# impromptuRong/hd_yolo

Hardware: AMD Instinct MI355X
Metric: tiles/sec (640x640) fwd+bwd (higher is better)
Workload: dtype bf16; 1 GPU; metayolo yolov5s 8-class nuclei, 640x640 RGB tiles, batch 64/GPU, train step = fwd + DetLoss + bwd + all-reduce + SGD(nesterov); global_batch=64, parallelism=dp1, world_size=1, backend=none, hw_queues=4

## Files before the change

### hd_yolo_amd/build.py

```python
import os
import subprocess
import sys
from concurrent.futures import ThreadPoolExecutor

HERE = os.path.dirname(os.path.abspath(__file__))
CSRC = os.path.join(HERE, 'csrc')
OUT = os.path.join(CSRC, 'build')
LIB = os.path.join(OUT, 'libhdyolo_hip.so')
SOURCES = ['api.hip', 'conv_dispatch.hip', 'conv_igemm.hip', 'conv3x3.hip', 'conv3x3_c128.hip', 'conv3x3s2.hip', 'conv_deep.hip', 'conv_stem.hip', 'conv_wgrad.hip', 'conv_wgrad3x3.hip', 'conv_wgrad_deep.hip', 'conv_dgrad_s2.hip', 'conv1x1_bwd.hip', 'bn_act.hip', 'pool.hip', 'detect.hip', 'nms_grid.hip', 'slide.hip', 'augment.hip', 'augment_masks.hip', 'score.hip', 'paste.hip', 'mask_score.hip', 'measure.hip', 'spatial.hip', 'outline.hip', 'graph.hip', 'loss.hip', 'roi.hip', 'seg.hip', 'optim.hip', 'exec.hip']
FLAGS = ['--offload-arch=gfx950', '-O3', '-fPIC', '-std=c++17', '-ffp-contract=off', '-Wall', '-Wno-unused-function',
         '-I' + CSRC, '-I' + os.path.join(os.path.dirname(HERE), 'include')]


def _newer(a, bs):
    return os.path.exists(a) and all(os.path.getmtime(a) >= os.path.getmtime(b) for b in bs)


def build(force=False, verbose=True):
    os.makedirs(OUT, exist_ok=True)
    headers = [os.path.join(CSRC, h) for h in os.listdir(CSRC) if h.endswith('.h')]
    headers += [os.path.join(os.path.dirname(HERE), 'include', h) for h in ('hdyolo.h', 'hdyolo_measure.h', 'hdyolo_spatial.h', 'hdyolo_outline.h', 'hdyolo_graph.h')]
    hipcc = os.environ.get('HIPCC', '/opt/rocm/bin/hipcc')

    def compile_one(src):
        s = os.path.join(CSRC, src)
        o = os.path.join(OUT, src.replace('.hip', '.o'))
        if not force and _newer(o, [s] + headers):
            return o
        cmd = [hipcc] + FLAGS + ['-c', s, '-o', o]
        if verbose:
            print(' '.join(cmd), flush=True)
        subprocess.check_call(cmd)
        return o

    with ThreadPoolExecutor(max_workers=min(6, os.cpu_count() or 1)) as ex:
        objs = list(ex.map(compile_one, SOURCES))
    if force or not _newer(LIB, objs):
        cmd = [hipcc, '--offload-arch=gfx950', '-shared', '-fPIC', '-o', LIB] + objs
        if verbose:
            print(' '.join(cmd), flush=True)
        subprocess.check_call(cmd)
    return LIB


if __name__ == '__main__':
    print(build(force='--force' in sys.argv))
```

### hd_yolo_amd/csrc/api.hip

```cpp
#include <stdarg.h>
#include <stdio.h>
#include <stdlib.h>
#include <string.h>

#include <atomic>

#include "common.h"
#include "hdyolo_internal.h"
#include "hdyolo.h"

int hdy_pack_weight_launch(const hdy_pack_desc& d, hipStream_t st);
int hdy_pack_batch_launch(const hdy_pack_desc* table, int n, int total_blocks, hipStream_t st);

static thread_local char g_err[512] = "";

void hdy_set_error(const char* fmt, ...) {
    va_list ap;
    va_start(ap, fmt);
    vsnprintf(g_err, sizeof(g_err), fmt, ap);
    va_end(ap);
}

namespace {
struct OptDef { const char* name; int def; bool flag; };
const OptDef g_opt_def[HDY_OPT_COUNT] = {
    {"HDY_NO_CLASS_WALK", 0, true}, {"HDY_NO_CONV3X3", 0, true}, {"HDY_C3_GRID", 0, false}, {"HDY_NO_CONV3X3S2", 0, false},
    {"HDY_NO_DGRAD_S2", 0, false}, {"HDY_TILE_INTERLEAVE", 1, false}, {"HDY_NO_BIG_TILES", 0, true}, {"HDY_NO_STEM_KERNEL", 0, true},
    {"HDY_WGRAD_BLOCKS", 512, false}, {"HDY_NO_STEM_WGRAD", 0, true}, {"HDY_NO_WGRAD3X3", 0, true}, 
    {"HDY_LOSS_GRID", 2048, false}, {"HDY_NO_DEEP", 0, true}, {"HDY_NO_WGRAD_DEEP", 0, true}, {"HDY_DEEP_BN", 0, false}, {"HDY_DEEP_DEBUG", 0, false}, {"HDY_DEEP_ALL", 1, false}, {"HDY_DEEP_MIN_TILES", 160, false}, {"HDY_DEEP_WALK", 2, false}, {"HDY_NO_BN_REDUCE4", 0, true},
    {"HDY_WGRAD_TILE", 0, false}, {"HDY_SPPF_NO_KEYS", 0, true}, {"HDY_WGRAD_DEEP_KMIN", 192, false}, {"HDY_NO_CONV3X3_C128", 0, true}, {"HDY_NO_F1X1_96", 0, true},
    {"HDY_AP_CHUNK", 0, false}, {"HDY_AP_NO_PRUNE", 0, true},
};
std::atomic<int> g_opt[HDY_OPT_COUNT];
std::once_flag g_opt_once;
void opt_init() {
    std::call_once(g_opt_once, [] {
        for (int i = 0; i < HDY_OPT_COUNT; ++i) {
            const char* v = getenv(g_opt_def[i].name);
            g_opt[i].store(v ? (g_opt_def[i].flag ? 1 : atoi(v)) : g_opt_def[i].def, std::memory_order_relaxed);
        }
    });
}
int opt_index(const char* name) {
    for (int i = 0; name && i < HDY_OPT_COUNT; ++i)
        if (!strcmp(name, g_opt_def[i].name)) return i;
    return -1;
}
thread_local char g_disp_last[64] = "";
std::mutex g_disp_mu;
char g_disp_log[32768] = "";
size_t g_disp_len = 0;
thread_local char g_disp_copy[32768] = "";
}

int hdy_opt(int id) {
    opt_init();
    return g_opt[id].load(std::memory_order_relaxed);
}

void hdy_note_dispatch(const char* what) {
    snprintf(g_disp_last, sizeof(g_disp_last), "%s", what);
    const size_t n = strlen(g_disp_last);
    std::lock_guard<std::mutex> lock(g_disp_mu);
    if (g_disp_len + n + 2 < sizeof(g_disp_log)) {
        memcpy(g_disp_log + g_disp_len, g_disp_last, n);
        g_disp_log[g_disp_len + n] = ';';
        g_disp_log[g_disp_len + n + 1] = 0;
        g_disp_len += n + 1;
    }
}

namespace {

enum { KIND_FWD = 0, KIND_DGRAD = 1, KIND_STEM = 2 };

inline int velems(int dtype) { return dtype == HDY_BF16 ? 8 : 4; }
inline int bke(int dtype) { return 8 * velems(dtype); }
inline size_t esize(int dtype) { return dtype == HDY_BF16 ? 2 : 4; }

inline size_t block_elems(int rows, int kd, int dtype) {
    const int bn = hdy_conv_bn_tile(rows);
    return (size_t)round_up(rows, bn) * round_up(kd, bke(dtype));
}

}

extern "C" {

const char* hdy_last_error(void) { return g_err; }

const char* hdy_last_dispatch(void) { return g_disp_last; }

const char* hdy_dispatch_log(void) {
    std::lock_guard<std::mutex> lock(g_disp_mu);
    memcpy(g_disp_copy, g_disp_log, g_disp_len + 1);
    return g_disp_copy;
}

void hdy_dispatch_log_reset(void) {
    std::lock_guard<std::mutex> lock(g_disp_mu);
    g_disp_log[0] = 0;
    g_disp_len = 0;
    g_disp_last[0] = 0;
}

int hdy_set_option(const char* name, int value) {
    const int i = opt_index(name);
    HDY_ARG(i >= 0, "set_option: unknown option %s", name ? name : "(null)");
    opt_init();
    return g_opt[i].exchange(value, std::memory_order_relaxed);
}

int hdy_get_option(const char* name) {
    const int i = opt_index(name);
    HDY_ARG(i >= 0, "get_option: unknown option %s", name ? name : "(null)");
    return hdy_opt(i);
}

int hdy_version(void) { return HDY_ABI_VERSION; }

int hdy_fastdiv_magic(unsigned d, unsigned* magic, int* shift) {
    HDY_ARG(d > 0 && magic && shift, "fastdiv_magic: d must be positive");
    hdy_magic(d, magic, shift);
    return HDY_OK;
}

int hdy_conv_out_dim(int in, int k, int stride, int pad) { return conv_out_dim(in, k, stride, pad); }

int hdy_conv_mtiles(long long M) { return (int)((M + 127) / 128); }

size_t hdy_conv_pack_elems(int K, int C, int R, int S, int stride, int pad, int kind, int dtype) {
    if (kind == KIND_FWD) return block_elems(K, R * S * C, dtype);
    if (kind == KIND_STEM) return block_elems(K, R * S * 4, dtype);
    if (stride == 1) return block_elems(C, R * S * K, dtype);
    size_t n = 0;
    for (int a = 0; a < 2; ++a)
        for (int b = 0; b < 2; ++b) {
            const Axis ah = class_axis(R, pad, a), aw = class_axis(S, pad, b);
            if (ah.taps && aw.taps) n += block_elems(C, ah.taps * aw.taps * K, dtype);
        }
    return n;
}

static hdy_pack_desc make_desc(const float* w_a, int K_a, const float* w_b, int K_b, void* out, int Kl, int C, int R, int S, int transpose,
                               int TH, int TW, int rbase, int rstep, int sbase, int sstep, int stem, int rows_total, int Kdp, int dtype,
                               int first_block) {
    hdy_pack_desc d = {};
    d.w_a = w_a; d.w_b = w_b; d.out = out; d.K_a = K_a; d.K_b = K_b; d.Kl = Kl; d.C = C; d.R = R; d.S = S; d.transpose = transpose;
    d.TH = TH; d.TW = TW; d.rbase = rbase; d.rstep = rstep; d.sbase = sbase; d.sstep = sstep; d.stem = stem; d.rows_total = rows_total;
    d.Kdp = Kdp; d.dtype = dtype; d.first_block = first_block;
    d.nblocks = cdiv((long long)rows_total * Kdp, 2048);
    return d;
}

int hdy_conv_pack_describe(const float* w_a, int K_a, const float* w_b, int K_b, int K, int C, int R, int S, int stride, int pad, int kind,
                           int dtype, void* out, hdy_pack_desc* descs, int first_block) {
    HDY_ARG(w_a && out && descs && K_a > 0 && K_b >= 0 && K >= K_a + K_b && C > 0 && R > 0 && S > 0, "conv_pack: bad args");
    HDY_ARG((K_b == 0) == (w_b == nullptr), "conv_pack: w_b / K_b mismatch");
    HDY_ARG(stride == 1 || stride == 2, "conv_pack: stride %d unsupported", stride);
    HDY_ARG(dtype == HDY_BF16 || dtype == HDY_F32, "conv_pack: unknown dtype %d", dtype);
    HDY_ARG(((long long)K + 256) * ((long long)R * S * ((long long)C + 256) + 64) < (1LL << 31), "conv_pack: weight too large for 32-bit packing indices");
    if (kind == KIND_FWD || kind == KIND_STEM) {
        const int stem = kind == KIND_STEM;
        HDY_ARG(!stem || (C == 3 && K_b == 0), "conv_pack: stem expects C == 3 and a single weight");
        const int kd = stem ? R * S * 4 : R * S * C;
        const int Kdp = round_up(kd, bke(dtype));
        const int rows_total = round_up(K, hdy_conv_bn_tile(K));
        descs[0] = make_desc(w_a, K_a, w_b, K_b, out, K, C, R, S, 0, R, stem ? 1 : S, 0, 1, 0, 1, stem, rows_total, Kdp, dtype, first_block);
        return 1;
    }
    HDY_ARG(kind == KIND_DGRAD, "conv_pack: unknown kind %d", kind);
    const int rows_total = round_up(C, hdy_conv_bn_tile(C));
    if (stride == 1) {
        const int Kdp = round_up(R * S * K, bke(dtype));
        descs[0] = make_desc(w_a, K_a, w_b, K_b, out, K, C, R, S, 1, R, S, R - 1, -1, S - 1, -1, 0, rows_total, Kdp, dtype, first_block);
        return 1;
    }
    size_t off = 0;
    int n = 0;
    for (int a = 0; a < 2; ++a)
        for (int b = 0; b < 2; ++b) {
            const Axis ah = class_axis(R, pad, a), aw = class_axis(S, pad, b);
            if (!ah.taps || !aw.taps) continue;
            const int Kdp = round_up(ah.taps * aw.taps * K, bke(dtype));
// ... 28 lines not shown
```

### hd_yolo_amd/csrc/common.h

```cpp
#pragma once
#include <hip/hip_runtime.h>
#include <stdint.h>
#include <stddef.h>

#include <mutex>

#define HDY_OK 0
#define HDY_EINVAL (-1)
#define HDY_EUNSUPPORTED (-2)

enum { HDY_F32 = 0, HDY_BF16 = 1 };

void hdy_set_error(const char* fmt, ...);

enum HdyOption {
    HDY_OPT_NO_CLASS_WALK,
    HDY_OPT_NO_CONV3X3,
    HDY_OPT_C3_GRID,
    HDY_OPT_NO_CONV3X3S2,
    HDY_OPT_NO_DGRAD_S2,
    HDY_OPT_TILE_INTERLEAVE,
    HDY_OPT_NO_BIG_TILES,
    HDY_OPT_NO_STEM_KERNEL,
    HDY_OPT_WGRAD_BLOCKS,
    HDY_OPT_NO_STEM_WGRAD,
    HDY_OPT_NO_WGRAD3X3,
    HDY_OPT_LOSS_GRID,
    HDY_OPT_NO_DEEP,
    HDY_OPT_NO_WGRAD_DEEP,
    HDY_OPT_DEEP_BN,
    HDY_OPT_DEEP_DEBUG,
    HDY_OPT_DEEP_ALL,
    HDY_OPT_DEEP_MIN_TILES,
    HDY_OPT_DEEP_WALK,
    HDY_OPT_NO_BN_REDUCE4,
    HDY_OPT_WGRAD_TILE,
    HDY_OPT_SPPF_NO_KEYS,
    HDY_OPT_WGRAD_DEEP_KMIN,
    HDY_OPT_NO_CONV3X3_C128,
    HDY_OPT_NO_F1X1_96,
    HDY_OPT_AP_CHUNK,
    HDY_OPT_AP_NO_PRUNE,
    HDY_OPT_COUNT
};
int hdy_opt(int id);

void hdy_note_dispatch(const char* what);

#define HDY_ARG(cond, ...)                 \
    do {                                   \
        if (!(cond)) {                     \
            hdy_set_error(__VA_ARGS__);    \
            return HDY_EINVAL;             \
        }                                  \
    } while (0)

#define HDY_LAUNCH_CHECK(what)                                                       \
    do {                                                                             \
        hipError_t e__ = hipGetLastError();                                          \
        if (e__ != hipSuccess) {                                                     \
            hdy_set_error("%s: launch failed: %s", what, hipGetErrorString(e__));    \
            return (int)e__;                                                         \
        }                                                                            \
    } while (0)

typedef __bf16 bf16_t;
typedef int i32x4 __attribute__((ext_vector_type(4)));
typedef float f32x4 __attribute__((ext_vector_type(4)));
typedef __bf16 bf16x8 __attribute__((ext_vector_type(8)));
typedef __bf16 bf16x4 __attribute__((ext_vector_type(4)));

#if defined(__HIPCC__)
__device__ __forceinline__ float row_sum16(float v) {
#ifdef HDY_ROW_SUM_SHFL
    for (int m = 1; m < 16; m <<= 1) v += __shfl_xor(v, m);
    return v;
#endif
    v += __builtin_bit_cast(float, __builtin_amdgcn_update_dpp(0, __builtin_bit_cast(int, v), 0x128, 0xF, 0xF, true));
    v += __builtin_bit_cast(float, __builtin_amdgcn_update_dpp(0, __builtin_bit_cast(int, v), 0x124, 0xF, 0xF, true));
    v += __builtin_bit_cast(float, __builtin_amdgcn_update_dpp(0, __builtin_bit_cast(int, v), 0x122, 0xF, 0xF, true));
    v += __builtin_bit_cast(float, __builtin_amdgcn_update_dpp(0, __builtin_bit_cast(int, v), 0x121, 0xF, 0xF, true));
    return v;
}
#endif

struct PerDeviceOnce {
    std::once_flag flag[16];
    template <typename F> void run(F&& fn) {
        int dev = 0;
        (void)hipGetDevice(&dev);
        std::call_once(flag[dev & 15], fn);
    }
};

static inline int cdiv(long long a, long long b) { return (int)((a + b - 1) / b); }
static inline int round_up(int a, int b) { return (a + b - 1) / b * b; }

#ifdef __HIPCC__
union V16 {
    i32x4 i;
    f32x4 f;
    bf16x8 h;
};

__device__ __forceinline__ float silu_f(float u) { return u / (1.0f + __expf(-u)); }
__device__ __forceinline__ float sigmoid_f(float u) { return 1.0f / (1.0f + __expf(-u)); }

template <typename T> __device__ __forceinline__ float to_f32(T v);
template <> __device__ __forceinline__ float to_f32<float>(float v) { return v; }
template <> __device__ __forceinline__ float to_f32<bf16_t>(bf16_t v) { return (float)v; }
template <typename T> __device__ __forceinline__ T from_f32(float v);
template <> __device__ __forceinline__ float from_f32<float>(float v) { return v; }
template <> __device__ __forceinline__ bf16_t from_f32<bf16_t>(float v) { return (bf16_t)v; }

__device__ __forceinline__ int xcd_remap(int id, int n) {
    const int q = n >> 3, r = n & 7, x = id & 7, s = id >> 3;
    return (x < r ? x * (q + 1) : r * (q + 1) + (x - r) * q) + s;
}
__device__ __forceinline__ unsigned fdiv(unsigned n, unsigned mg, int sh) { return __umulhi(n << 1, mg) >> sh; }

__device__ __forceinline__ bool iou_gt(float ax1, float ay1, float ax2, float ay2, float aarea, float bx1, float by1, float bx2, float by2,
                                       float barea, float thr) {
    const float xx1 = ax1 > bx1 ? ax1 : bx1;
    const float yy1 = ay1 > by1 ? ay1 : by1;
    const float xx2 = ax2 < bx2 ? ax2 : bx2;
    const float yy2 = ay2 < by2 ? ay2 : by2;
    float w = __fsub_rn(xx2, xx1);
    float h = __fsub_rn(yy2, yy1);
    w = w < 0.f ? 0.f : w;
    h = h < 0.f ? 0.f : h;
    const float inter = __fmul_rn(w, h);
    const float ovr = __fdiv_rn(inter, __fsub_rn(__fadd_rn(aarea, barea), inter));
    return ovr > thr;
}

__device__ __forceinline__ unsigned desc_key(float s) {
    unsigned u = s == 0.0f ? 0u : __float_as_uint(s);
    u = (u & 0x80000000u) ? ~u : (u | 0x80000000u);
    return ~u;
}

__device__ __forceinline__ void glds16(const void* g, unsigned char* lds_wave_base) {
    __builtin_amdgcn_global_load_lds((const void __attribute__((address_space(1)))*)g,
                                     (void __attribute__((address_space(3)))*)lds_wave_base, 16, 0, 0);
}

__device__ __forceinline__ void lds_dma16(__amdgpu_buffer_rsrc_t r, unsigned voff, unsigned soff, unsigned char* lds_wave_base) {
    __builtin_amdgcn_raw_ptr_buffer_load_lds(r, (void __attribute__((address_space(3)))*)lds_wave_base, 16, (int)voff, (int)soff, 0, 0);
}

__device__ __forceinline__ void lds_dma16(__amdgpu_buffer_rsrc_t r, unsigned voff, unsigned soff, unsigned lds_byte) {
    __builtin_amdgcn_raw_ptr_buffer_load_lds(r, (void __attribute__((address_space(3)))*)(uintptr_t)lds_byte, 16, (int)voff, (int)soff, 0, 0);
}

__device__ __forceinline__ int fsw(int row) { return ((row >> 1) & 1) | (((row >> 3) & 1) << 1); }
__device__ __forceinline__ int fsw3(int row) { return (row & 6) ^ (((row >> 3) & 1) * 5); }

__device__ __forceinline__ float fast_sigmoid(float u) { return __builtin_amdgcn_rcpf(1.0f + __expf(-u)); }
__device__ __forceinline__ float dsilu_f(float u) {
    const float s = fast_sigmoid(u);
    return s * (1.0f + u * (1.0f - s));
}

template <typename T> __device__ __forceinline__ void unpack(const i32x4& v, float* f);
template <> __device__ __forceinline__ void unpack<float>(const i32x4& v, float* f) {
    V16 u; u.i = v;
#pragma unroll
    for (int i = 0; i < 4; ++i) f[i] = u.f[i];
}
template <> __device__ __forceinline__ void unpack<bf16_t>(const i32x4& v, float* f) {
    V16 u; u.i = v;
#pragma unroll
    for (int i = 0; i < 8; ++i) f[i] = (float)u.h[i];
}
template <typename T> __device__ __forceinline__ i32x4 pack(const float* f);
template <> __device__ __forceinline__ i32x4 pack<float>(const float* f) {
    V16 u;
#pragma unroll
    for (int i = 0; i < 4; ++i) u.f[i] = f[i];
    return u.i;
}
template <> __device__ __forceinline__ i32x4 pack<bf16_t>(const float* f) {
    V16 u;
#pragma unroll
    for (int i = 0; i < 8; ++i) u.h[i] = (bf16_t)f[i];
    return u.i;
}

#define VEC_OK(ptr, ld, VE) ((((uintptr_t)(ptr)) & 15) == 0 && (ld) % (VE) == 0)

#define S2_LDSR(dst, addr)                                                                             \
    do {                                                                                               \
        if constexpr (HAND) asm volatile("ds_read_b128 %0, %1" : "=v"(dst) : "v"(addr) : "memory");    \
        else dst = *(const i32x4*)(smem + ((addr) - lds0));                                            \
    } while (0)
// ... 11 lines not shown
```

### hd_yolo_amd/csrc/conv_dispatch.hip

```cpp
#include "common.h"
#include "hdyolo_internal.h"
#include "hdyolo.h"

static inline int bke(int dtype) { return dtype == HDY_BF16 ? 64 : 32; }

static ConvPlan conv_fwd_plan(const ConvShape& s, int first = CONV_STEM) {
    ConvPlan p = {};
    if (first <= CONV_STEM && hdy_conv_stem_plan(s, &p)) return p;
    if (first <= CONV_3X3_C64 && hdy_conv3x3_c64_plan(s, &p)) return p;
    if (first <= CONV_3X3_C128 && hdy_conv3x3_c128_plan(s, &p)) return p;
    if (first <= CONV_3X3S2 && hdy_conv3x3s2_plan(s, &p)) return p;
    if (first <= CONV_DGRAD_S2 && hdy_dgrad3x3s2_plan(s, &p)) return p;
    if (first <= CONV_DEEP && hdy_conv_deep_plan(s, &p)) return p;
    hdy_conv_igemm_plan(s, &p);
    return p;
}

extern "C" int hdy_conv_stat_slabs(int N, int H, int W, int C, int K, int R, int S, int stride, int pad, int dtype) {
    const int stem = C == 3 && R == 6 && S == 6 && stride == 2 && pad == 2;
    return conv_fwd_plan(conv_shape(N, H, W, C, K, R, S, stride, pad, dtype, stem, 1)).slabs;
}

static int launch_planned(const ConvArgs& a, const ConvPlan& p, int dtype, int out_f32, hipStream_t st) {
    switch (p.family) {
        case CONV_STEM: return hdy_conv_stem_launch(a, p, out_f32, st);
        case CONV_3X3_C64: return hdy_conv3x3_c64_launch(a, p, out_f32, st);
        case CONV_3X3_C128: return hdy_conv3x3_c128_launch(a, p, out_f32, st);
        case CONV_3X3S2: return hdy_conv3x3s2_launch(a, p, out_f32, st);
        case CONV_DGRAD_S2: return hdy_dgrad3x3s2_launch(a, p, out_f32, st);
        case CONV_DEEP: return hdy_conv_deep_launch(a, p, out_f32, st);
        default: return hdy_conv_igemm_launch(a, p, dtype, out_f32, st);
    }
}

static int hdy_conv_launch(ConvArgs a, const ConvShape& s, int out_f32, hipStream_t st) {
    const int dtype = s.dtype;
    const int VE = dtype == HDY_BF16 ? 8 : 4;
    HDY_ARG(a.x && a.w && a.y, "conv: null pointer");
    HDY_ARG(a.N > 0 && a.Hin > 0 && a.Win > 0 && a.Ho > 0 && a.Wo > 0 && a.K > 0 && a.C > 0, "conv: non-positive dim");
    HDY_ARG(a.C % VE == 0, "conv: C=%d must be a multiple of %d for this dtype", a.C, VE);
    HDY_ARG(a.ldx % (a.span_pixels ? 4 : VE) == 0 && (a.span_pixels || a.ldx >= a.C), "conv: ldx=%d must be >= C and a multiple of %d", a.ldx, VE);
    HDY_ARG(a.ldy >= a.K, "conv: ldy=%d < K=%d", a.ldy, a.K);
    HDY_ARG(((uintptr_t)a.x & 15) == 0 && ((uintptr_t)a.w & 15) == 0, "conv: x/w must be 16-byte aligned");
    HDY_ARG(a.TH > 0 && a.TW > 0, "conv: empty tap window");
    HDY_ARG(a.Hin < 24000 && a.Win < 24000 && a.TH < 64 && a.TW < 64 && a.dh0 > -4000 && a.dw0 > -4000, "conv: image side beyond the loader's 16-bit coordinates");
    HDY_ARG((long long)a.N * a.Hin * a.Win < (1LL << 31) && (long long)a.N * a.Ho * a.Wo < (1LL << 31), "conv: too many pixels");
    a.Kd = a.TH * a.TW * a.C;
    const int BKE = 8 * VE;
    a.bn = hdy_conv_bn_tile(a.K);
    HDY_ARG(a.Kdp == round_up(a.Kd, BKE), "conv: packed weight pitch %d != %d", a.Kdp, round_up(a.Kd, BKE));
    a.M = a.N * a.Ho * a.Wo;
    a.mtiles = cdiv(a.M, 128);
    a.ntiles = cdiv(a.K, a.bn);
    if (a.dense_out) HDY_ARG(a.oh_mul == 1 && a.ow_mul == 1 && a.oh_off == 0 && a.ow_off == 0 && a.Hout == a.Ho && a.Wout == a.Wo, "conv: dense_out geometry mismatch");
    a.pointwise = (a.TH == 1 && a.TW == 1 && a.ih_mul == 1 && a.iw_mul == 1 && a.dh0 == 0 && a.dw0 == 0 && a.Hin == a.Ho && a.Win == a.Wo &&
                   !a.span_pixels && a.ncls <= 1) ? 1 : 0;
    if (a.ncls > 1) {
        HDY_ARG(a.ncls == 4 && !a.dense_out && !a.stats, "conv: class walk is the four-class stride-2 dgrad");
        for (int c = 0; c < 4; ++c) HDY_ARG(a.c_nkb[c] == round_up(a.c_TH[c] * a.c_TW[c] * a.C, BKE) / BKE, "conv: class %d k-blocks", c);
    }
    const bool bf16_out = dtype == HDY_BF16 && !out_f32;
    a.vec_out = (bf16_out && a.K % 8 == 0 && a.ldy % 8 == 0 && ((uintptr_t)a.y & 15) == 0 &&
                 (!a.res || (a.ldr % 8 == 0 && ((uintptr_t)a.res & 15) == 0))) ? 1 : 0;
    if (a.nstat > 0) {
        HDY_ARG(a.nstat <= 2 && a.vec_out && a.ntiles == 1 && a.bn <= 64 && !a.stats && !a.res, "conv: producer-side statistics need the bf16 vector epilogue and at most 64 output channels");
        for (int r = 0; r < a.nstat; ++r) {
            const StatReq& q = a.stat[r];
            HDY_ARG(q.y && q.scale && q.shift && q.slabs && q.c0 >= 0 && q.c0 < q.c1 && q.c1 <= a.K && q.c0 % 8 == 0 && q.c1 % 8 == 0 &&
                    q.ldy % 8 == 0 && (((uintptr_t)q.y | (uintptr_t)q.scale | (uintptr_t)q.shift) & 15) == 0,
                    "conv: bad statistics request %d", r);
        }
    }
    a.uh0 = a.dh0; a.uw0 = a.dw0;
    int uh1 = a.dh0 + a.TH, uw1 = a.dw0 + a.TW;
    for (int c = 0; c < (a.ncls > 1 ? 4 : 0); ++c) {
        a.uh0 = a.c_dh[c] < a.uh0 ? a.c_dh[c] : a.uh0; a.uw0 = a.c_dw[c] < a.uw0 ? a.c_dw[c] : a.uw0;
        uh1 = a.c_dh[c] + a.c_TH[c] > uh1 ? a.c_dh[c] + a.c_TH[c] : uh1; uw1 = a.c_dw[c] + a.c_TW[c] > uw1 ? a.c_dw[c] + a.c_TW[c] : uw1;
    }
    a.UH = uh1 - a.uh0; a.UW = uw1 - a.uw0;
    HDY_ARG(a.UH * a.UW <= 31, "conv: %d x %d tap window beyond the loader's 31 tap bits", a.UH, a.UW);
    HDY_ARG(((long long)(a.UH + 1) * a.Win + a.UW) * a.ldx * (dtype == HDY_BF16 ? 2 : 4) < (1LL << 28), "conv: tap window spans too many bytes");
    a.utap = a.C % BKE == 0 ? 1 : 0;
    hdy_magic((unsigned)(a.Ho * a.Wo), &a.mg_howo, &a.sh_howo);
    hdy_magic((unsigned)a.Wo, &a.mg_wo, &a.sh_wo);
    hdy_magic((unsigned)a.C, &a.mg_c, &a.sh_c);
    for (int c = 0; c < 4; ++c) hdy_magic((unsigned)(a.ncls > 1 ? a.c_TW[c] : a.TW), &a.mg_tw[c], &a.sh_tw[c]);
    for (int first = a.nstat > 0 ? CONV_IGEMM : CONV_STEM;;) {
        const ConvPlan p = conv_fwd_plan(s, first);
        a.tile_interleave = p.interleave;
        const int rc = launch_planned(a, p, dtype, out_f32, st);
        if (rc != HDY_CONV_DECLINE) return rc;
        first = p.family + 1;
    }
}

static bool dgrad_class_walk(int H, int W, int R, int S, int pad) {
    if (H % 2 || W % 2 || hdy_opt(HDY_OPT_NO_CLASS_WALK)) return false;
    for (int a = 0; a < 2; ++a)
        if (!class_axis(R, pad, a).taps || !class_axis(S, pad, a).taps) return false;
    return true;
}

static ConvShape dgrad_shape(int N, int H, int W, int C, int K, int R, int S, int stride, int pad, int dtype) {
    const bool walk = stride == 2;
    const int pad1 = R == S && pad <= R - 1 ? R - 1 - pad : -1;
    return ConvShape{N, conv_out_dim(H, R, stride, pad), conv_out_dim(W, S, stride, pad), H / stride, W / stride, K, C, R, S, stride, walk ? pad : pad1,
                     !walk, dtype, 0, 0, walk ? 4 : 1};
}

static int dgrad_impl(const void* dy, int lddy, const void* w_packed_dgrad, void* dx, int lddx, int N, int H, int W, int C, int K, int R,
                      int S, int stride, int pad, int accumulate, int dtype, const hdy_stat_req* stats, int nstat, void* stream) {
    HDY_ARG(stride == 1 || stride == 2, "conv_dgrad: stride %d unsupported", stride);
    HDY_ARG(dtype == HDY_BF16 || dtype == HDY_F32, "conv_dgrad: unknown dtype %d", dtype);
    const int Ho = conv_out_dim(H, R, stride, pad), Wo = conv_out_dim(W, S, stride, pad);
    HDY_ARG(Ho > 0 && Wo > 0, "conv_dgrad: empty dy");
    ConvArgs a = {};
    a.x = dy; a.y = dx; a.N = N; a.Hin = Ho; a.Win = Wo; a.C = K; a.ldx = lddy;
    a.K = C; a.ldy = lddx; a.Hout = H; a.Wout = W;
    a.ih_mul = a.iw_mul = 1; a.accumulate = accumulate;
    a.nstat = nstat;
    for (int r = 0; r < nstat; ++r)
        a.stat[r] = StatReq{stats[r].y, stats[r].ldy, stats[r].scale, stats[r].shift, stats[r].slabs, stats[r].c0, stats[r].c1, stats[r].act, stats[r].nslabs};
    if (stride == 1) {
        a.w = w_packed_dgrad;
        a.Ho = H; a.Wo = W; a.oh_mul = a.ow_mul = 1; a.dense_out = 1;
        a.dh0 = pad - (R - 1); a.dw0 = pad - (S - 1); a.TH = R; a.TW = S;
        a.Kdp = round_up(R * S * K, bke(dtype));
        return hdy_conv_launch(a, dgrad_shape(N, H, W, C, K, R, S, stride, pad, dtype), 0, (hipStream_t)stream);
    }
    const int rows_total = round_up(C, hdy_conv_bn_tile(C));
    size_t off = 0;
    if (dgrad_class_walk(H, W, R, S, pad)) {
        ConvArgs c = a;
        c.ncls = 4;
        c.Ho = H / 2; c.Wo = W / 2;
        c.oh_mul = c.ow_mul = 2; c.dense_out = 0;
        for (int ca = 0; ca < 2; ++ca)
            for (int cb = 0; cb < 2; ++cb) {
                const Axis ah = class_axis(R, pad, ca), aw = class_axis(S, pad, cb);
                const int i = ca * 2 + cb;
                const int Kdp = round_up(ah.taps * aw.taps * K, bke(dtype));
                c.c_dh[i] = ah.d0; c.c_dw[i] = aw.d0; c.c_TH[i] = ah.taps; c.c_TW[i] = aw.taps;
                c.c_nkb[i] = Kdp / bke(dtype); c.c_oh[i] = ca; c.c_ow[i] = cb; c.c_w[i] = (long long)off;
                off += (size_t)rows_total * Kdp;
            }
        c.w = w_packed_dgrad;
        c.dh0 = c.c_dh[0]; c.dw0 = c.c_dw[0]; c.TH = c.c_TH[0]; c.TW = c.c_TW[0]; c.oh_off = c.ow_off = 0;
        c.Kdp = c.c_nkb[0] * bke(dtype);
        return hdy_conv_launch(c, dgrad_shape(N, H, W, C, K, R, S, stride, pad, dtype), 0, (hipStream_t)stream);
    }
    for (int ca = 0; ca < 2; ++ca)
        for (int cb = 0; cb < 2; ++cb) {
            const Axis ah = class_axis(R, pad, ca), aw = class_axis(S, pad, cb);
            ConvArgs c = a;
            c.Ho = (H - ca + 1) / 2; c.Wo = (W - cb + 1) / 2;
            c.oh_mul = c.ow_mul = 2; c.oh_off = ca; c.ow_off = cb; c.dense_out = 0;
            if (!ah.taps || !aw.taps) {
                HDY_ARG(false, "conv_dgrad: kernel %dx%d pad %d leaves a parity class without taps (unsupported)", R, S, pad);
            }
            if (c.Ho <= 0 || c.Wo <= 0) continue;
            c.dh0 = ah.d0; c.dw0 = aw.d0; c.TH = ah.taps; c.TW = aw.taps;
            c.Kdp = round_up(ah.taps * aw.taps * K, bke(dtype));
            c.w = (const char*)w_packed_dgrad + off * (dtype == HDY_BF16 ? 2 : 4);
            off += (size_t)rows_total * c.Kdp;
            const ConvShape s = {N, Ho, Wo, c.Ho, c.Wo, K, C, ah.taps, aw.taps, 1, -1, 0, dtype, 0, 0, 1};
            const int rc = hdy_conv_launch(c, s, 0, (hipStream_t)stream);
            if (rc) return rc;
        }
    return HDY_OK;
}

extern "C" {

int hdy_conv_fwd(const void* x, int ldx, const void* w_packed, const float* scale, const float* shift, const void* res, int ldr, void* y,
                 int ldy, float* stats, int stat_slabs, int N, int H, int W, int C, int K, int R, int S, int stride, int pad, int act, int accumulate,
                 int dtype, int out_f32, int stem, void* stream) {
    HDY_ARG(!stats || stat_slabs > 0, "conv_fwd: stats given with stat_slabs = %d", stat_slabs);
    HDY_ARG(stride >= 1 && R >= 1 && S >= 1 && pad >= 0, "conv_fwd: bad window");
    HDY_ARG(dtype == HDY_BF16 || dtype == HDY_F32, "conv_fwd: unknown dtype %d", dtype);
    ConvArgs a = {};
    a.x = x; a.w = w_packed; a.y = y; a.scale = scale; a.shift = shift; a.stats = stats; a.stat_cap = stat_slabs; a.res = res; a.ldr = ldr;
    HDY_ARG(!res || ldr >= K, "conv_fwd: residual pitch %d < K", ldr);
// ... 133 lines not shown
```

### hd_yolo_amd/csrc/hdyolo_internal.h

```cpp
#pragma once
#include <type_traits>

#include "common.h"

struct StatReq {
    const void* y; int ldy;
    const float *scale, *shift;
    float* slabs;
    int c0, c1, act;
    int nslabs;
};

struct ConvArgs {
    const void* x;
    const void* w;
    void* y;
    const float* scale;
    const float* shift;
    float* stats;
    int stat_cap;
    const void* res;
    int ldr;
    int N, Hin, Win, C, ldx;
    int Ho, Wo, K, ldy;
    int Hout, Wout, oh_mul, oh_off, ow_mul, ow_off;
    int ih_mul, iw_mul, dh0, dw0, TH, TW;
    int Kd, Kdp, M;
    int act, accumulate, dense_out;
    int mtiles, ntiles, bn;
    int span_pixels;
    int pointwise;
    int vec_out;
    int nstat;
    StatReq stat[2];
    int ncls;
    int c_dh[4], c_dw[4], c_TH[4], c_TW[4], c_nkb[4], c_oh[4], c_ow[4];
    long long c_w[4];
    int uh0, uw0, UH, UW, utap;
    int tile_interleave;
    unsigned mg_howo, mg_wo, mg_c, mg_tw[4];
    int sh_howo, sh_wo, sh_c, sh_tw[4];
    int dbg;
};

struct ConvShape {
    int N, H, W;
    int Ho, Wo;
    int C, K, R, S, stride;
    int pad;
    int dense;
    int dtype;
    int stem;
    int stats;
    int ncls;
};
inline int hdy_conv_bn_tile(int K) { return K <= 32 ? 32 : (K <= 64 ? 64 : 128); }
inline int conv_out_dim(int in, int k, int stride, int pad) { return (in + 2 * pad - k) / stride + 1; }
struct Axis { int taps, d0, rmax; };
inline Axis class_axis(int R, int pad, int a) {
    Axis ax = {0, 0, -1};
    for (int r = R - 1; r >= 0; --r)
        if (((a + pad - r) & 1) == 0) {
            if (ax.rmax < 0) { ax.rmax = r; ax.d0 = (a + pad - r) / 2; }
            ++ax.taps;
        }
    return ax;
}
inline ConvShape conv_shape(int N, int H, int W, int C, int K, int R, int S, int stride, int pad, int dtype, int stem, int stats) {
    return ConvShape{N, H, W, conv_out_dim(H, R, stride, pad), conv_out_dim(W, S, stride, pad), C, K, R, S, stride, pad, 1, dtype, stem, stats, 1};
}
inline long long conv_pixels(const ConvShape& s) { return (long long)s.N * s.Ho * s.Wo; }
inline int conv_taps(const ConvShape& s) { return s.stem ? 6 : s.R * s.S; }
inline bool conv_is(const ConvShape& s, int R, int stride, int pad) { return !s.stem && s.ncls <= 1 && s.R == R && s.S == R && s.stride == stride && s.pad == pad; }

enum ConvFamily { CONV_NONE = 0, CONV_STEM, CONV_3X3_C64, CONV_3X3_C128, CONV_3X3S2, CONV_DGRAD_S2, CONV_DEEP, CONV_IGEMM };

struct ConvPlan {
    int family;
    int variant;
    int grid;
    int slabs;
    int bn;
    int interleave;
};

bool hdy_conv_stem_plan(const ConvShape& s, ConvPlan* p);
bool hdy_conv3x3_c64_plan(const ConvShape& s, ConvPlan* p);
bool hdy_conv3x3_c128_plan(const ConvShape& s, ConvPlan* p);
bool hdy_conv3x3s2_plan(const ConvShape& s, ConvPlan* p);
bool hdy_dgrad3x3s2_plan(const ConvShape& s, ConvPlan* p);
bool hdy_conv_deep_plan(const ConvShape& s, ConvPlan* p);
bool hdy_conv_igemm_plan(const ConvShape& s, ConvPlan* p);

enum { HDY_CONV_DECLINE = -100 };
int hdy_conv_stem_launch(const ConvArgs& a, const ConvPlan& p, int out_f32, hipStream_t st);
int hdy_conv3x3_c64_launch(const ConvArgs& a, const ConvPlan& p, int out_f32, hipStream_t st);
int hdy_conv3x3_c128_launch(const ConvArgs& a, const ConvPlan& p, int out_f32, hipStream_t st);
int hdy_conv3x3s2_launch(const ConvArgs& a, const ConvPlan& p, int out_f32, hipStream_t st);
int hdy_dgrad3x3s2_launch(const ConvArgs& a, const ConvPlan& p, int out_f32, hipStream_t st);
int hdy_conv_deep_launch(const ConvArgs& a, const ConvPlan& p, int out_f32, hipStream_t st);
int hdy_conv_igemm_launch(const ConvArgs& a, const ConvPlan& p, int dtype, int out_f32, hipStream_t st);

inline int hdy_conv_take(const ConvArgs& a, const ConvPlan& p, bool fits, const char* who) {
    if (!fits && !a.stats) return HDY_CONV_DECLINE;
    HDY_ARG(fits, "%s: statistics requested, but this call does not fit the kernel their slabs were sized for (bf16 output, 16-byte aligned x/y/res rows; "
            "ldx=%d ldy=%d)", who, a.ldx, a.ldy);
    HDY_ARG(!a.stats || a.stat_cap == p.slabs, "%s: the statistics array holds %d slabs, this launch writes %d (a kernel-selection option changed between "
            "hdy_conv_stat_slabs and the launch?)", who, a.stat_cap, p.slabs);
    return HDY_OK;
}

inline bool rows_aligned(const ConvArgs& a, bool need_w) {
    return a.ldx % 8 == 0 && a.ldy % 8 == 0 && (((uintptr_t)a.x | (uintptr_t)a.y) & 15) == 0 && (!need_w || (((uintptr_t)a.w & 15) == 0 && a.Kdp % 8 == 0)) &&
           (!a.res || (a.ldr % 8 == 0 && ((uintptr_t)a.res & 15) == 0));
}

inline int epilogue_of(const ConvArgs& a) { return a.act == 1 ? 2 : ((a.scale || a.shift) ? 1 : 0); }

template <typename F> inline void with_stats_epi(bool stats, int epi, F&& f) {
    auto with_epi = [&](auto s) {
        if (epi == 2) f(s, std::integral_constant<int, 2>{});
        else if (epi == 1) f(s, std::integral_constant<int, 1>{});
        else f(s, std::integral_constant<int, 0>{});
    };
    if (stats) with_epi(std::true_type{});
    else with_epi(std::false_type{});
}

inline int hdy_launch_status(const char* who) {
    HDY_LAUNCH_CHECK(who);
    return HDY_OK;
}

inline void hdy_magic(unsigned d, unsigned* mg, int* sh) {
    int s = 0;
    while ((1ull << s) < d) ++s;
    *mg = (unsigned)((((unsigned long long)1 << (31 + s)) + d - 1) / d);
    *sh = s;
}

struct WgradArgs {
    const void* x;
    const void* dy;
    float* partial;
    int N, Hin, Win, C, ldx;
    int Ho, Wo, K, lddy;
    int ih_mul, iw_mul, dh0, dw0, TH, TW;
    int Q, P;
    int splits, pix_per_split;
    int ktiles, qtiles;
    int span_pixels;
    const void* y; int ldy;
    const float *bn_scale, *bn_shift, *bn_mean, *bn_invstd, *bn_c1, *bn_c2;
};

struct WgradShape {
    int N, H, W;
    int Ho, Wo;
    int C, K, R, S, stride, pad, dtype;
    int stem;
};
inline WgradShape wgrad_shape(int N, int H, int W, int C, int K, int R, int S, int stride, int pad, int dtype, int stem) {
    return WgradShape{N, H, W, conv_out_dim(H, R, stride, pad), conv_out_dim(W, S, stride, pad), C, K, R, S, stride, pad, dtype, stem};
}
inline long long wgrad_pixels(const WgradShape& s) { return (long long)s.N * s.Ho * s.Wo; }
inline int wgrad_cols(const WgradShape& s) { return s.R * s.S * (s.stem ? 4 : s.C); }

enum WgradFamily { WGRAD_STEM, WGRAD_3X3, WGRAD_DEEP, WGRAD_GENERIC };

struct WgradPlan {
    int family;
    int variant;
    int grid;
    int splits;
    int pix_per_split;
    int ktiles, qtiles;
    int TOH, TOW, tiles_h, tiles_w;
};

bool hdy_wgrad_stem_plan(const WgradShape& s, WgradPlan* p);
bool hdy_wgrad3x3_plan(const WgradShape& s, WgradPlan* p);
bool hdy_wgrad_deep_plan(const WgradShape& s, WgradPlan* p);
bool hdy_wgrad_generic_plan(const WgradShape& s, WgradPlan* p);

int hdy_wgrad_stem_launch(const WgradArgs& a, const WgradPlan& p, hipStream_t st);
int hdy_wgrad3x3_launch(const WgradArgs& a, const WgradPlan& p, hipStream_t st);
int hdy_wgrad_deep_launch(const WgradArgs& a, const WgradPlan& p, hipStream_t st);
int hdy_wgrad_generic_launch(const WgradArgs& a, const WgradPlan& p, hipStream_t st);
int hdy_wgrad_reduce(const float* partial, int splits, int K, int Q, int mode, int C, int R, int S, float* grad_a, int K_a, float* grad_b, int K_b,
                     int accumulate, hipStream_t st);
```

Before: 5590 tiles/s.

## Add dedicated persistent 1x1 convolution kernel with LDS ring pipeline

```diff
diff --git a/hd_yolo_amd/build.py b/hd_yolo_amd/build.py
--- a/hd_yolo_amd/build.py
+++ b/hd_yolo_amd/build.py
@@ -7,7 +7,7 @@
 CSRC = os.path.join(HERE, 'csrc')
 OUT = os.path.join(CSRC, 'build')
 LIB = os.path.join(OUT, 'libhdyolo_hip.so')
-SOURCES = ['api.hip', 'conv_dispatch.hip', 'conv_igemm.hip', 'conv3x3.hip', 'conv3x3_c128.hip', 'conv3x3s2.hip', 'conv_deep.hip', 'conv_stem.hip', 'conv_wgrad.hip', 'conv_wgrad3x3.hip', 'conv_wgrad_deep.hip', 'conv_dgrad_s2.hip', 'conv1x1_bwd.hip', 'bn_act.hip', 'pool.hip', 'detect.hip', 'nms_grid.hip', 'slide.hip', 'augment.hip', 'augment_masks.hip', 'score.hip', 'paste.hip', 'mask_score.hip', 'measure.hip', 'spatial.hip', 'outline.hip', 'graph.hip', 'loss.hip', 'roi.hip', 'seg.hip', 'optim.hip', 'exec.hip']
+SOURCES = ['api.hip', 'conv_dispatch.hip', 'conv_igemm.hip', 'conv3x3.hip', 'conv3x3_c128.hip', 'conv1x1.hip', 'conv3x3s2.hip', 'conv_deep.hip', 'conv_stem.hip', 'conv_wgrad.hip', 'conv_wgrad3x3.hip', 'conv_wgrad_deep.hip', 'conv_dgrad_s2.hip', 'conv1x1_bwd.hip', 'bn_act.hip', 'pool.hip', 'detect.hip', 'nms_grid.hip', 'slide.hip', 'augment.hip', 'augment_masks.hip', 'score.hip', 'paste.hip', 'mask_score.hip', 'measure.hip', 'spatial.hip', 'outline.hip', 'graph.hip', 'loss.hip', 'roi.hip', 'seg.hip', 'optim.hip', 'exec.hip']
 FLAGS = ['--offload-arch=gfx950', '-O3', '-fPIC', '-std=c++17', '-ffp-contract=off', '-Wall', '-Wno-unused-function',
          '-I' + CSRC, '-I' + os.path.join(os.path.dirname(HERE), 'include')]
 
diff --git a/hd_yolo_amd/csrc/api.hip b/hd_yolo_amd/csrc/api.hip
--- a/hd_yolo_amd/csrc/api.hip
+++ b/hd_yolo_amd/csrc/api.hip
@@ -29,7 +29,7 @@
     {"HDY_WGRAD_BLOCKS", 512, false}, {"HDY_NO_STEM_WGRAD", 0, true}, {"HDY_NO_WGRAD3X3", 0, true}, 
     {"HDY_LOSS_GRID", 2048, false}, {"HDY_NO_DEEP", 0, true}, {"HDY_NO_WGRAD_DEEP", 0, true}, {"HDY_DEEP_BN", 0, false}, {"HDY_DEEP_DEBUG", 0, false}, {"HDY_DEEP_ALL", 1, false}, {"HDY_DEEP_MIN_TILES", 160, false}, {"HDY_DEEP_WALK", 2, false}, {"HDY_NO_BN_REDUCE4", 0, true},
     {"HDY_WGRAD_TILE", 0, false}, {"HDY_SPPF_NO_KEYS", 0, true}, {"HDY_WGRAD_DEEP_KMIN", 192, false}, {"HDY_NO_CONV3X3_C128", 0, true}, {"HDY_NO_F1X1_96", 0, true},
-    {"HDY_AP_CHUNK", 0, false}, {"HDY_AP_NO_PRUNE", 0, true},
+    {"HDY_AP_CHUNK", 0, false}, {"HDY_AP_NO_PRUNE", 0, true}, {"HDY_NO_CONV1X1", 0, true}, {"HDY_CONV1X1_MIN_PIXELS", 98304, false}, {"HDY_CONV1X1_GRID", 0, false},
 };
 std::atomic<int> g_opt[HDY_OPT_COUNT];
 std::once_flag g_opt_once;
diff --git a/hd_yolo_amd/csrc/common.h b/hd_yolo_amd/csrc/common.h
--- a/hd_yolo_amd/csrc/common.h
+++ b/hd_yolo_amd/csrc/common.h
@@ -41,6 +41,9 @@
     HDY_OPT_NO_F1X1_96,
     HDY_OPT_AP_CHUNK,
     HDY_OPT_AP_NO_PRUNE,
+    HDY_OPT_NO_CONV1X1,
+    HDY_OPT_CONV1X1_MIN_PIXELS,
+    HDY_OPT_CONV1X1_GRID,
     HDY_OPT_COUNT
 };
 int hdy_opt(int id);
diff --git a/hd_yolo_amd/csrc/conv1x1.hip b/hd_yolo_amd/csrc/conv1x1.hip
--- /dev/null
+++ b/hd_yolo_amd/csrc/conv1x1.hip
@@ -0,0 +1,283 @@
+#include <stdio.h>
+#include <stdlib.h>
+
+#include <type_traits>
+
+#include "common.h"
+#include "hdyolo_internal.h"
+
+__device__ uint4 g_hdy_zero16_c1[4];
+
+namespace {
+
+typedef int i32x2 __attribute__((ext_vector_type(2)));
+
+constexpr int NW = 8, NTHR = NW * 64;
+constexpr int TILE_B = 16384;
+constexpr int NR = 6;
+constexpr int LPT = TILE_B / 1024 / NW;
+constexpr int MAX_GRID = 256;
+
+template <int C, int K> struct Geo {
+    static constexpr int CB = C * 2, CPP = C / 8, KS = C / 32;
+    static constexpr int TP = TILE_B / CB;
+    static constexpr int KW = K >= 128 ? 32 : 16, KF = KW / 16;
+    static constexpr int KG = K / KW, PG = NW / KG;
+    static constexpr int FW = TP / 16 / PG;
+    static constexpr int NG = FW * KS;
+    static constexpr int KB = K * 2, CPR = K / 8;
+    static constexpr int RPP = NTHR / CPR, NST = TP / RPP;
+    static constexpr int STAGE_B = TP * KB;
+    static constexpr int SMEM_B = NR * TILE_B + STAGE_B;
+    static_assert(KG * PG == NW && FW >= 1 && FW * PG * 16 == TP && NG <= 16 && NST >= 1 && NST * RPP == TP, "conv1x1: instance geometry");
+    static_assert(SMEM_B <= 160 * 1024 && PG * 2 * K * 4 <= NR * TILE_B, "conv1x1: LDS");
+};
+
+template <int CB> __host__ __device__ constexpr int in_key(int p) { return CB >= 256 ? (p & 15) : (CB == 128 ? ((p >> 1) & 7) : ((0 - (p >> 2)) & 3)); }
+template <int KB> __host__ __device__ constexpr int out_key(int p) { return KB >= 128 ? (p & 15) : ((p >> 1) & 7); }
+
+#define C1_VM(n) case n: asm volatile("s_waitcnt vmcnt(" #n ")" ::: "memory"); break;
+__device__ __forceinline__ void wait_vm(int n) {
+    switch (n < 48 ? n : 48) {
+        C1_VM(0) C1_VM(1) C1_VM(2) C1_VM(3) C1_VM(4) C1_VM(5) C1_VM(6) C1_VM(7) C1_VM(8) C1_VM(9) C1_VM(10) C1_VM(11) C1_VM(12) C1_VM(13) C1_VM(14) C1_VM(15)
+        C1_VM(16) C1_VM(17) C1_VM(18) C1_VM(19) C1_VM(20) C1_VM(21) C1_VM(22) C1_VM(23) C1_VM(24) C1_VM(25) C1_VM(26) C1_VM(27) C1_VM(28) C1_VM(29) C1_VM(30) C1_VM(31)
+        C1_VM(32) C1_VM(33) C1_VM(34) C1_VM(35) C1_VM(36) C1_VM(37) C1_VM(38) C1_VM(39) C1_VM(40) C1_VM(41) C1_VM(42) C1_VM(43) C1_VM(44) C1_VM(45) C1_VM(46) C1_VM(47)
+        default: asm volatile("s_waitcnt vmcnt(48)" ::: "memory"); break;
+    }
+}
+#undef C1_VM
+
+#define C1_BARRIER() do { asm volatile("s_waitcnt lgkmcnt(0)" ::: "memory"); __builtin_amdgcn_s_barrier(); asm volatile("" ::: "memory"); } while (0)
+
+template <int C, int K, bool STATS, bool ACC>
+__global__ __launch_bounds__(NTHR, 1) void conv1x1_kernel(const ConvArgs p, const int nslabs) {
+    using G = Geo<C, K>;
+    constexpr int CB = G::CB, CPP = G::CPP, KS = G::KS, TP = G::TP, KW = G::KW, KF = G::KF, KG = G::KG, FW = G::FW, NG = G::NG, KB = G::KB, CPR = G::CPR,
+                  RPP = G::RPP, NST = G::NST;
+    constexpr int NSTQ = ACC ? 2 * NST : NST;
+    extern __shared__ __attribute__((aligned(16))) unsigned char smem[];
+    const unsigned lds0 = (unsigned)(uintptr_t)(const __attribute__((address_space(3))) unsigned char*)smem;
+    const unsigned stage0 = lds0 + NR * TILE_B;
+
+    const int tid = threadIdx.x, lane = tid & 63, wave = tid >> 6;
+    const int fr = lane & 15, fq = lane >> 4;
+    const int kg = wave % KG, pg = wave / KG;
+    const int ngrid = (int)gridDim.x, wg = xcd_remap(blockIdx.x, ngrid);
+    const int tiles = (p.M + TP - 1) / TP, per = tiles / ngrid, rem = tiles - per * ngrid;
+    const int n = per + (wg < rem ? 1 : 0), t0 = wg * per + (wg < rem ? wg : rem);
+
+    const bf16_t* __restrict__ x = (const bf16_t*)p.x;
+    const bf16_t* __restrict__ w = (const bf16_t*)p.w;
+    const unsigned char* zero = (const unsigned char*)g_hdy_zero16_c1;
+
+    V16 bw[KF][KS];
+#pragma unroll
+    for (int kf = 0; kf < KF; ++kf)
+#pragma unroll
+        for (int ks = 0; ks < KS; ++ks) {
+            i32x4 v_;
+            asm volatile("global_load_dwordx4 %0, %1, off" : "=v"(v_) : "v"(w + (size_t)(kg * KW + kf * 16 + fr) * p.Kdp + (ks * 4 + fq) * 8) : "memory");
+            bw[kf][ks].i = v_;
+        }
+
+    int lrel[LPT], lpix[LPT];
+#pragma unroll
+    for (int i = 0; i < LPT; ++i) {
+        const int d = (i * NW + wave) * 64 + lane;
+        const int pt = d / CPP, ph = d % CPP;
+        lpix[i] = pt;
+        lrel[i] = pt * p.ldx + ((ph ^ in_key<CB>(pt)) << 3);
+    }
+    auto issue_tile = [&](int t, int slot) {
+        const long long pix0 = (long long)t * TP;
+        const bf16_t* org = x + pix0 * p.ldx;
+#pragma unroll
+        for (int i = 0; i < LPT; ++i) {
+            const void* src = pix0 + lpix[i] < p.M ? (const void*)(org + lrel[i]) : (const void*)zero;
+            glds16(src, smem + slot * TILE_B + (i * NW + wave) * 1024);
+        }
+    };
+
+    unsigned boff[KS], swo[KF];
+#pragma unroll
+    for (int ks = 0; ks < KS; ++ks) boff[ks] = lds0 + (pg * FW * 16 + fr) * CB + (((ks * 4 + fq) ^ in_key<CB>(fr)) << 4);
+#pragma unroll
+    for (int kf = 0; kf < KF; ++kf) swo[kf] = stage0 + (pg * FW * 16 + fr) * KB + (((kg * (KW / 4) + kf * 4 + fq) ^ out_key<KB>(fr)) << 3);
+    const int st_c = tid % CPR, st_r = tid / CPR, st_key = out_key<KB>(st_r);
+    const unsigned srd = stage0 + st_r * KB + ((st_c ^ (st_key >> 1)) << 4);
+
+    float s1[KF][4], s2[KF][4];
+#pragma unroll
+    for (int kf = 0; kf < KF; ++kf)
+#pragma unroll
+        for (int r = 0; r < 4; ++r) s1[kf][r] = s2[kf][r] = 0.f;
+
+    int issued = 0;
+    for (; issued < n && issued < NR - 1; ++issued) issue_tile(t0 + issued, issued);
+
+    for (int s = 0; s < n; ++s) {
+        wait_vm((issued - 1 - s) * LPT + (s < NR - 1 ? s : NR - 1) * NSTQ);
+#pragma unroll
+        for (int kf = 0; kf < KF; ++kf)
+#pragma unroll
+            for (int ks = 0; ks < KS; ++ks) asm volatile("" : "+v"(bw[kf][ks].i));
+        C1_BARRIER();
+        if (issued < n) {
+            issue_tile(t0 + issued, issued % NR);
+            ++issued;
+        }
+        const unsigned tb = (unsigned)((s % NR) * TILE_B);
+        V16 fa[NG];
+#pragma unroll
+        for (int g = 0; g < NG; ++g) {
+            i32x4 v_;
+            asm volatile("ds_read_b128 %0, %1 offset:%2" : "=v"(v_) : "v"(boff[g % KS] + tb), "n"((g / KS) * 16 * CB));
+            fa[g].i = v_;
+        }
+        f32x4 acc[FW][KF];
+#pragma unroll
+        for (int j = 0; j < FW; ++j)
+#pragma unroll
+            for (int kf = 0; kf < KF; ++kf) acc[j][kf] = f32x4{0.f, 0.f, 0.f, 0.f};
+#pragma unroll
+        for (int g = 0; g < NG; ++g) {
+            asm volatile("s_waitcnt lgkmcnt(%1)" : "+v"(fa[g].i) : "n"(NG - 1 - g));
+#pragma unroll
+            for (int kf = 0; kf < KF; ++kf) acc[g / KS][kf] = __builtin_amdgcn_mfma_f32_16x16x32_bf16(bw[kf][g % KS].h, fa[g].h, acc[g / KS][kf], 0, 0, 0);
+        }
+        if (STATS) {
+#pragma unroll
+            for (int j = 0; j < FW; ++j)
+#pragma unroll
+                for (int kf = 0; kf < KF; ++kf)
+#pragma unroll
+                    for (int r = 0; r < 4; ++r) {
+                        const float v = acc[j][kf][r];
+                        s1[kf][r] += v;
+                        s2[kf][r] = __builtin_fmaf(v, v, s2[kf][r]);
+                    }
+        }
+#pragma unroll
+        for (int j = 0; j < FW; ++j)
+#pragma unroll
+            for (int kf = 0; kf < KF; ++kf) {
+                const bf16x4 o = {(bf16_t)acc[j][kf][0], (bf16_t)acc[j][kf][1], (bf16_t)acc[j][kf][2], (bf16_t)acc[j][kf][3]};
+                asm volatile("ds_write_b64 %0, %1 offset:%2" ::"v"(swo[kf]), "v"(__builtin_bit_cast(i32x2, o)), "n"(j * 16 * KB) : "memory");
+            }
+        C1_BARRIER();
+        i32x4 ov[NST];
+#pragma unroll
+        for (int i = 0; i < NST; ++i) asm volatile("ds_read_b128 %0, %1 offset:%2" : "=v"(ov[i]) : "v"(srd), "n"(i * RPP * KB));
+        const long long row0 = (long long)(t0 + s) * TP + st_r;
+        bf16_t* yb = (bf16_t*)p.y + row0 * p.ldy + st_c * 8;
+#pragma unroll
+        for (int i = 0; i < NST; ++i) {
+            asm volatile("s_waitcnt lgkmcnt(%1)" : "+v"(ov[i]) : "n"(NST - 1 - i));
+            if (row0 + i * RPP < p.M) {
+                V16 v;
+                v.i = ov[i];
+                if (st_key & 1) v.i = i32x4{v.i[2], v.i[3], v.i[0], v.i[1]};
+                bf16_t* dst = yb + (long long)i * RPP * p.ldy;
+                if (ACC) {
+                    V16 q;
+                    q.i = *(const i32x4*)dst;
+#pragma unroll
+                    for (int e = 0; e < 8; ++e) v.h[e] = (bf16_t)((float)v.h[e] + (float)q.h[e]);
+                }
+                *(i32x4*)dst = v.i;
+            }
+        }
+    }
+
+    if (STATS) {
+        __syncthreads();
+        float* red = (float*)smem;
+#pragma unroll
+        for (int kf = 0; kf < KF; ++kf)
+#pragma unroll
+            for (int r = 0; r < 4; ++r) {
+                const float u = row_sum16(s1[kf][r]), q = row_sum16(s2[kf][r]);
+                const int c = kg * KW + kf * 16 + fq * 4 + r;
+                if (fr == 0) {
+                    red[(pg * 2 + 0) * K + c] = u;
+                    red[(pg * 2 + 1) * K + c] = q;
+                }
+            }
+        __syncthreads();
+        if (tid < 2 * K) {
+            float u = 0.f;
+#pragma unroll
+            for (int g = 0; g < G::PG; ++g) u += red[g * 2 * K + tid];
+            p.stats[(size_t)wg * 2 * K + tid] = u;
+            for (int slab = ngrid + wg; slab < nslabs; slab += ngrid) p.stats[(size_t)slab * 2 * K + tid] = 0.f;
+        }
+    }
+}
+
+template <int C, int K, bool STATS, bool ACC>
+static void launch_c1(const ConvArgs& a, int grid, hipStream_t st) {
+    constexpr int smem_b = Geo<C, K>::SMEM_B;
+    static PerDeviceOnce attr_once;
+    attr_once.run([&] {
+        (void)hipFuncSetAttribute((const void*)conv1x1_kernel<C, K, STATS, ACC>, hipFuncAttributeMaxDynamicSharedMemorySize, smem_b);
+    });
+    hipLaunchKernelGGL((conv1x1_kernel<C, K, STATS, ACC>), dim3(grid), dim3(NTHR), smem_b, st, a, a.stats ? a.stat_cap : 0);
+}
+
+template <int C, int K>
+static void launch_c1_ck(const ConvArgs& a, int grid, hipStream_t st) {
+    if (a.stats) launch_c1<C, K, true, false>(a, grid, st);
+    else if (a.accumulate) launch_c1<C, K, false, true>(a, grid, st);
+    else launch_c1<C, K, false, false>(a, grid, st);
+}
+
+constexpr int variant_of(int C, int K) { return C * 1024 + K; }
+inline bool has_instance(int C, int K) {
+    switch (variant_of(C, K)) {
+        case variant_of(32, 32): case variant_of(32, 64): case variant_of(64, 32): case variant_of(64, 64): case variant_of(64, 128): case variant_of(128, 64):
+        case variant_of(128, 128): case variant_of(128, 256): case variant_of(256, 128): case variant_of(256, 256): return true;
+        default: return false;
+    }
+}
+
+}
+
+bool hdy_conv1x1_plan(const ConvShape& s, ConvPlan* p) {
+    if (hdy_opt(HDY_OPT_NO_CONV1X1) || s.dtype != HDY_BF16 || !conv_is(s, 1, 1, 0) || !s.dense || !has_instance(s.C, s.K)) return false;
+    if (hdy_opt(HDY_OPT_DEEP_MIN_TILES) < 160 || hdy_opt(HDY_OPT_DEEP_BN)) return false;
+    const long long M = conv_pixels(s);
+    if (M < hdy_opt(HDY_OPT_CONV1X1_MIN_PIXELS) || M >= (1LL << 31)) return false;
+    const long long tiles = (M + TILE_B / (2 * s.C) - 1) / (TILE_B / (2 * s.C));
+    const int cap = hdy_opt(HDY_OPT_CONV1X1_GRID) > 0 && hdy_opt(HDY_OPT_CONV1X1_GRID) < MAX_GRID ? hdy_opt(HDY_OPT_CONV1X1_GRID) : MAX_GRID;
+    int grid = tiles < cap ? (int)tiles : cap;
+    ConvPlan after = {};
+    if (!hdy_conv_deep_plan(s, &after)) hdy_conv_igemm_plan(s, &after);
+    if (s.stats && after.slabs < grid) {
+        if (tiles >= MAX_GRID) return false;
+        grid = after.slabs;
+    }
+    *p = ConvPlan{CONV_1X1, variant_of(s.C, s.K), grid, after.slabs, 0, 0};
+    return true;
+}
+
+int hdy_conv1x1_launch(const ConvArgs& a, const ConvPlan& p, int out_f32, hipStream_t st) {
+    const bool raw = !out_f32 && epilogue_of(a) == 0 && a.act == 0 && !a.res && !(a.stats && a.accumulate) && a.nstat == 0;
+    if (const int rc = hdy_conv_take(a, p, raw && a.pointwise && rows_aligned(a, true), "conv1x1")) return rc;
+    HDY_ARG(!a.stats || (p.grid >= 1 && p.grid <= p.slabs), "conv1x1: %d workgroups for %d statistic slabs", p.grid, p.slabs);
+    char name[32];
+    snprintf(name, sizeof(name), "conv1x1_c%dk%d", a.C, a.K);
+    hdy_note_dispatch(name);
+    switch (p.variant) {
+        case variant_of(32, 32): launch_c1_ck<32, 32>(a, p.grid, st); break;
+        case variant_of(32, 64): launch_c1_ck<32, 64>(a, p.grid, st); break;
+        case variant_of(64, 32): launch_c1_ck<64, 32>(a, p.grid, st); break;
+        case variant_of(64, 64): launch_c1_ck<64, 64>(a, p.grid, st); break;
+        case variant_of(64, 128): launch_c1_ck<64, 128>(a, p.grid, st); break;
+        case variant_of(128, 64): launch_c1_ck<128, 64>(a, p.grid, st); break;
+        case variant_of(128, 128): launch_c1_ck<128, 128>(a, p.grid, st); break;
+        case variant_of(128, 256): launch_c1_ck<128, 256>(a, p.grid, st); break;
+        case variant_of(256, 128): launch_c1_ck<256, 128>(a, p.grid, st); break;
+        default: launch_c1_ck<256, 256>(a, p.grid, st); break;
+    }
+    return hdy_launch_status("conv1x1");
+}
diff --git a/hd_yolo_amd/csrc/conv_dispatch.hip b/hd_yolo_amd/csrc/conv_dispatch.hip
--- a/hd_yolo_amd/csrc/conv_dispatch.hip
+++ b/hd_yolo_amd/csrc/conv_dispatch.hip
@@ -11,6 +11,7 @@
     if (first <= CONV_3X3_C128 && hdy_conv3x3_c128_plan(s, &p)) return p;
     if (first <= CONV_3X3S2 && hdy_conv3x3s2_plan(s, &p)) return p;
     if (first <= CONV_DGRAD_S2 && hdy_dgrad3x3s2_plan(s, &p)) return p;
+    if (first <= CONV_1X1 && hdy_conv1x1_plan(s, &p)) return p;
     if (first <= CONV_DEEP && hdy_conv_deep_plan(s, &p)) return p;
     hdy_conv_igemm_plan(s, &p);
     return p;
@@ -28,6 +29,7 @@
         case CONV_3X3_C128: return hdy_conv3x3_c128_launch(a, p, out_f32, st);
         case CONV_3X3S2: return hdy_conv3x3s2_launch(a, p, out_f32, st);
         case CONV_DGRAD_S2: return hdy_dgrad3x3s2_launch(a, p, out_f32, st);
+        case CONV_1X1: return hdy_conv1x1_launch(a, p, out_f32, st);
         case CONV_DEEP: return hdy_conv_deep_launch(a, p, out_f32, st);
         default: return hdy_conv_igemm_launch(a, p, dtype, out_f32, st);
     }
diff --git a/hd_yolo_amd/csrc/hdyolo_internal.h b/hd_yolo_amd/csrc/hdyolo_internal.h
--- a/hd_yolo_amd/csrc/hdyolo_internal.h
+++ b/hd_yolo_amd/csrc/hdyolo_internal.h
@@ -73,7 +73,7 @@
 inline int conv_taps(const ConvShape& s) { return s.stem ? 6 : s.R * s.S; }
 inline bool conv_is(const ConvShape& s, int R, int stride, int pad) { return !s.stem && s.ncls <= 1 && s.R == R && s.S == R && s.stride == stride && s.pad == pad; }
 
-enum ConvFamily { CONV_NONE = 0, CONV_STEM, CONV_3X3_C64, CONV_3X3_C128, CONV_3X3S2, CONV_DGRAD_S2, CONV_DEEP, CONV_IGEMM };
+enum ConvFamily { CONV_NONE = 0, CONV_STEM, CONV_3X3_C64, CONV_3X3_C128, CONV_3X3S2, CONV_DGRAD_S2, CONV_1X1, CONV_DEEP, CONV_IGEMM };
 
 struct ConvPlan {
     int family;
@@ -89,6 +89,7 @@
 bool hdy_conv3x3_c128_plan(const ConvShape& s, ConvPlan* p);
 bool hdy_conv3x3s2_plan(const ConvShape& s, ConvPlan* p);
 bool hdy_dgrad3x3s2_plan(const ConvShape& s, ConvPlan* p);
+bool hdy_conv1x1_plan(const ConvShape& s, ConvPlan* p);
 bool hdy_conv_deep_plan(const ConvShape& s, ConvPlan* p);
 bool hdy_conv_igemm_plan(const ConvShape& s, ConvPlan* p);
 
@@ -98,6 +99,7 @@
 int hdy_conv3x3_c128_launch(const ConvArgs& a, const ConvPlan& p, int out_f32, hipStream_t st);
 int hdy_conv3x3s2_launch(const ConvArgs& a, const ConvPlan& p, int out_f32, hipStream_t st);
 int hdy_dgrad3x3s2_launch(const ConvArgs& a, const ConvPlan& p, int out_f32, hipStream_t st);
+int hdy_conv1x1_launch(const ConvArgs& a, const ConvPlan& p, int out_f32, hipStream_t st);
 int hdy_conv_deep_launch(const ConvArgs& a, const ConvPlan& p, int out_f32, hipStream_t st);
 int hdy_conv_igemm_launch(const ConvArgs& a, const ConvPlan& p, int dtype, int out_f32, hipStream_t st);
 
```

After: 5656 tiles/s, median of 6. 1.2% higher.
